# learningmatter-mit/surface-sampling

Hardware: AMD Instinct MI355X
Metric: MC energy-evaluations/sec (SrTiO3(001) ~250-atom slabs, 3-model PaiNN ensemble E+F incl. neighbor list) (higher is better)
Workload: dtype f32 via fp16x2-split MFMA (3 products), fp32 accumulate; neighbor decisions f64; 1 GPU; SrTiO3(001) PaiNN x3, 256 batched independent chains per GPU (BASELINE configs[3]), 248-272 atoms/chain; chains_per_gpu=256, atoms_per_gpu=66503, edges_per_gpu=2747786, slots_per_gpu=2836316, models=3, streams_per_gpu=2, parallelism=one GPU, no collective

## Files before the change

surface-sampling_amd/csrc/api_batch.hip:

```cpp
#include <cmath>

#include "ewald_dev.h"

namespace vssr {

static void cell_host_setup(const double *cell, const uint8_t *pbc, double cutoff, double inv[9], int nimg[3],
                            bool &ok) {
    const double *a = cell, *b = cell + 3, *c = cell + 6;
    double bc[3] = {b[1] * c[2] - b[2] * c[1], b[2] * c[0] - b[0] * c[2], b[0] * c[1] - b[1] * c[0]};
    double ca[3] = {c[1] * a[2] - c[2] * a[1], c[2] * a[0] - c[0] * a[2], c[0] * a[1] - c[1] * a[0]};
    double ab[3] = {a[1] * b[2] - a[2] * b[1], a[2] * b[0] - a[0] * b[2], a[0] * b[1] - a[1] * b[0]};
    double vol = a[0] * bc[0] + a[1] * bc[1] + a[2] * bc[2];
    ok = true;
    for (int x = 0; x < 9; ++x) inv[x] = 0.0;
    nimg[0] = nimg[1] = nimg[2] = 0;
    if (!(pbc[0] || pbc[1] || pbc[2])) return;
    if (std::fabs(vol) < 1e-12) { ok = false; return; }
    for (int x = 0; x < 3; ++x) { inv[x] = bc[x] / vol; inv[3 + x] = ca[x] / vol; inv[6 + x] = ab[x] / vol; }
    double hgt[3] = {std::fabs(vol) / std::sqrt(bc[0] * bc[0] + bc[1] * bc[1] + bc[2] * bc[2]),
                     std::fabs(vol) / std::sqrt(ca[0] * ca[0] + ca[1] * ca[1] + ca[2] * ca[2]),
                     std::fabs(vol) / std::sqrt(ab[0] * ab[0] + ab[1] * ab[1] + ab[2] * ab[2])};
    for (int k = 0; k < 3; ++k)
        if (pbc[k]) nimg[k] = (int)std::floor(cutoff / hgt[k]) + 1;
}
// ... 66 lines not shown
        }
        h->ew_stride = (int)stride;
        if (h->d_ew_S.ensure(sizeof(double) * 2 * (size_t)n_cfg * (size_t)(stride + 1)))
            return set_err(h, VSSR_E_NOMEM, "k-space structure factors: out of device memory");
    }
    if (h->d_pos.ensure(sizeof(double) * 3 * N) || h->d_Z.ensure(sizeof(int) * N) ||
        h->d_atom_cfg.ensure(sizeof(int) * N) || h->d_cfg_start.ensure(sizeof(int) * (n_cfg + 1)) ||
        h->d_cell.ensure(sizeof(double) * 9 * n_cfg) || h->d_invcell.ensure(sizeof(double) * 9 * n_cfg) ||
        h->d_nimg.ensure(sizeof(int) * 3 * n_cfg) || h->d_pbc.ensure((size_t)3 * n_cfg))
        return set_err(h, VSSR_E_NOMEM, "batch buffers: out of device memory");
    VSSR_HIP(h, hipMemcpy(h->d_pos.p, pos, sizeof(double) * 3 * N, hipMemcpyHostToDevice));
    VSSR_HIP(h, hipMemcpy(h->d_Z.p, Z, sizeof(int) * N, hipMemcpyHostToDevice));
    VSSR_HIP(h, hipMemcpy(h->d_atom_cfg.p, atom_cfg.data(), sizeof(int) * N, hipMemcpyHostToDevice));
    VSSR_HIP(h, hipMemcpy(h->d_cfg_start.p, start.data(), sizeof(int) * (n_cfg + 1), hipMemcpyHostToDevice));
    VSSR_HIP(h, hipMemcpy(h->d_cell.p, cell, sizeof(double) * 9 * n_cfg, hipMemcpyHostToDevice));
    VSSR_HIP(h, hipMemcpy(h->d_invcell.p, inv.data(), sizeof(double) * 9 * n_cfg, hipMemcpyHostToDevice));
    VSSR_HIP(h, hipMemcpy(h->d_nimg.p, nimg.data(), sizeof(int) * 3 * n_cfg, hipMemcpyHostToDevice));
    VSSR_HIP(h, hipMemcpy(h->d_pbc.p, pbc, (size_t)3 * n_cfg, hipMemcpyHostToDevice));
    h->n_cfg = n_cfg;
    h->n_atoms = N;
    if (h->kind == Kind::PAINN) {
        std::vector<int> zmap(h->n_embed, -1), zlist;
        for (int i = 0; i < N; ++i)
            if (zmap[Z[i]] < 0) { zmap[Z[i]] = 1; }
        for (int z = 0; z < h->n_embed; ++z)
            if (zmap[z] > 0) { zmap[z] = (int)zlist.size(); zlist.push_back(z); }
        h->l0_nz = (int)zlist.size() <= L0_MAX_SPECIES ? (int)zlist.size() : 0;
        if (h->d_zmap.ensure(sizeof(int) * h->n_embed) || h->d_zlist.ensure(sizeof(int) * (zlist.size() + 1)))
            return set_err(h, VSSR_E_NOMEM, "species tables");
        VSSR_HIP(h, hipMemcpy(h->d_zmap.p, zmap.data(), sizeof(int) * h->n_embed, hipMemcpyHostToDevice));
        VSSR_HIP(h, hipMemcpy(h->d_zlist.p, zlist.data(), sizeof(int) * zlist.size(), hipMemcpyHostToDevice));
    }
    h->max_cfg_atoms = 0;
    for (int b = 0; b < n_cfg; ++b) h->max_cfg_atoms = n_atoms[b] > h->max_cfg_atoms ? n_atoms[b] : h->max_cfg_atoms;
    if (h->kind == Kind::PAINN) {
        const bool bundles = (size_t)h->max_cfg_atoms * sizeof(int) <= 48 * 1024;
        std::vector<unsigned char> bcls(n_cfg);
        std::vector<int> lists[EDGE_MFMA_CLASSES], blists[EDGE_MFMA_BCLASSES];
        for (int c = 0; c < EDGE_CLASSES; ++c) { h->n_class[c] = 0; h->max_class_atoms[c] = 0; }
        for (int c = 0; c < EDGE_BCLASSES; ++c) { h->n_bclass[c] = 0; h->max_bclass_atoms[c] = 0; }
        for (int b = 0; b < n_cfg; ++b) {
            int c = (h->edge_impl && bundles) ? edge_class_of(n_atoms[b]) : EDGE_CLASS_GATHER;
            int bc = (h->edge_impl && bundles) ? edge_bclass_of(n_atoms[b]) : EDGE_BCLASS_GATHER;
            if (c <= EDGE_CLASS_FS16M && h->fs16_max_atoms >= 0 && n_atoms[b] > h->fs16_max_atoms) c = EDGE_CLASS_FS8;
            if (bc == EDGE_BCLASS_FS16 && h->fs16_max_atoms >= 0 && n_atoms[b] > h->fs16_max_atoms) bc = EDGE_BCLASS_FS8;
            if (c == EDGE_CLASS_FS8 && h->fs8_max_atoms >= 0 && n_atoms[b] > h->fs8_max_atoms) { c = EDGE_CLASS_FS4; bc = EDGE_BCLASS_FS4; }
            if (h->fwd_two_pass == 16 && c == EDGE_CLASS_FS8 && edge_class_of(n_atoms[b]) == EDGE_CLASS_FS8) c = EDGE_CLASS_FS4;
            if (bc != EDGE_BCLASS_GATHER && ((h->bwd_multi_pass == 1 && edge_bclass_of(n_atoms[b]) != EDGE_BCLASS_FS16) || h->bwd_multi_pass == 2))
                bc = EDGE_BCLASS_FS16P;
            bcls[b] = (unsigned char)bc;
            h->n_class[c] += 1;
            h->n_bclass[bc] += 1;
            if (n_atoms[b] > h->max_class_atoms[c]) h->max_class_atoms[c] = n_atoms[b];
            if (n_atoms[b] > h->max_bclass_atoms[bc]) h->max_bclass_atoms[bc] = n_atoms[b];
            if (c != EDGE_CLASS_GATHER) lists[c].push_back(b);
            if (bc != EDGE_BCLASS_GATHER) blists[bc].push_back(b);
        }
        std::vector<int> cat;
        for (int c = 0; c < EDGE_MFMA_CLASSES; ++c) cat.insert(cat.end(), lists[c].begin(), lists[c].end());
        for (int c = 0; c < EDGE_MFMA_BCLASSES; ++c) cat.insert(cat.end(), blists[c].begin(), blists[c].end());
        cat.push_back(0);
        const std::vector<unsigned char> &cls = bcls;
        if (h->d_chain_class.ensure((size_t)n_cfg) || h->d_class_list.ensure(sizeof(int) * cat.size()))
            return set_err(h, VSSR_E_NOMEM, "chain class tables");
        VSSR_HIP(h, hipMemcpy(h->d_chain_class.p, cls.data(), (size_t)n_cfg, hipMemcpyHostToDevice));
        VSSR_HIP(h, hipMemcpy(h->d_class_list.p, cat.data(), sizeof(int) * cat.size(), hipMemcpyHostToDevice));
    }
// ... 492 lines not shown
```

surface-sampling_amd/csrc/api_painn.hip:

```cpp
#include <cmath>

#include "vssr_internal.h"

namespace vssr {

static void transpose(const float *src, int rows, int cols, float *dst) {
    for (int r = 0; r < rows; ++r)
        for (int c = 0; c < cols; ++c) dst[(size_t)c * rows + r] = src[(size_t)r * cols + c];
}

static int upload_weights(vssr_handle *h, const vssr_painn_config *cfg) {
    const int M = cfg->n_models, L = cfg->num_conv, R = cfg->n_rbf, H = cfg->readout_hidden, NE = cfg->n_embed;
    const size_t per_layer = (size_t)F * F + F + (size_t)F3 * F + F3 + (size_t)F3 * R + F3 + 2 * (size_t)F * F +
                             (size_t)F * 2 * F + F + (size_t)F3 * F + F3;
    const size_t blob_len = (size_t)NE * F + L * per_layer + (size_t)H * F + H + H + 1;
    if (cfg->weights_len != blob_len)
        return set_err(h, VSSR_E_BADARG, "weights_len %llu does not match the layout (%zu floats)",
                       (unsigned long long)cfg->weights_len, blob_len);
    const size_t t_per_layer = (size_t)F * F + (size_t)F * F3 + 2 * (size_t)F * F + (size_t)2 * F * F + (size_t)F * F3;
    const size_t img_len = blob_len + L * t_per_layer + (size_t)F * H;
    std::vector<float> img(img_len * M);
    std::vector<ModelW> table(M);
    if (h->weights.ensure(img.size() * sizeof(float)))
        return set_err(h, VSSR_E_NOMEM, "weights: out of device memory");
// ... 104 lines not shown
            const float *W1 = hb + o; o += (size_t)F * F;
            const float *b1 = hb + o; o += F;
            const float *W2 = hb + o; o += (size_t)F3 * F;
            const float *b2 = hb + o; o += F3;
            const float *Wd = hb + o; o += (size_t)F3 * R;
            const float *bd = hb + o;
            l0_build_tables(hb, W1, b1, W2, b2, Wd, bd, NE, A.data() + per_model * m, At.data() + per_model * m);
        }
        const size_t pk = l0_packed_dwords(NE);
        std::vector<unsigned> A16(pk * M), At16(pk * M);
        for (int m = 0; m < M; ++m) l0_pack_tables(A.data() + per_model * m, NE, A16.data() + pk * m, At16.data() + pk * m);
        if (h->d_l0A.ensure(A16.size() * sizeof(unsigned)) || h->d_l0At.ensure(At16.size() * sizeof(unsigned)))
            return set_err(h, VSSR_E_NOMEM, "layer-0 tables");
        VSSR_HIP(h, hipMemcpy(h->d_l0A.p, A16.data(), A16.size() * sizeof(unsigned), hipMemcpyHostToDevice));
        VSSR_HIP(h, hipMemcpy(h->d_l0At.p, At16.data(), At16.size() * sizeof(unsigned), hipMemcpyHostToDevice));
    }
    if (h->model_table.ensure(sizeof(ModelW) * M)) return set_err(h, VSSR_E_NOMEM, "model table");
    VSSR_HIP(h, hipMemcpy(h->model_table.p, table.data(), sizeof(ModelW) * M, hipMemcpyHostToDevice));
    return VSSR_OK;
}

static void read_env_knobs(vssr_handle *h) {
    if (const char *e = getenv("VSSR_PAINN_PATH")) h->painn_general = h->painn_general || strcmp(e, "general") == 0;
    if (const char *e = getenv("VSSR_EDGE_IMPL")) h->edge_impl = (strcmp(e, "gather") == 0) ? 0 : 1;
    if (const char *e = getenv("VSSR_L0_FACTORISE")) h->l0_enabled = atoi(e);
    if (h->painn_general) h->l0_enabled = 0;
    if (const char *e = getenv("VSSR_UPD_SAVE")) h->upd_save = atoi(e);
    if (const char *e = getenv("VSSR_DEBUG_KEEP")) h->debug_keep = atoi(e);
    if (const char *e = getenv("VSSR_EDGE_FS16_MAX")) h->fs16_max_atoms = atoi(e);
    if (const char *e = getenv("VSSR_EDGE_FS8_MAX")) h->fs8_max_atoms = atoi(e);
    if (const char *e = getenv("VSSR_EDGE_BWD_MPASS")) h->bwd_multi_pass = atoi(e);
    if (const char *e = getenv("VSSR_EDGE_SUB_CHUNK")) { const int c = atoi(e); if (c >= 8) { h->sub_chunk_fwd = c; h->sub_chunk_bwd = c; } }
    if (const char *e = getenv("VSSR_EDGE_FWD_2PASS")) { const int w = atoi(e); h->fwd_two_pass = (w == 8 || w == 16) ? w : w ? 16 : 0; }
}

}

using namespace vssr;

extern "C" {

int vssr_create(const vssr_painn_config *cfg, vssr_handle **out) {
    if (!cfg || !out) return set_err(nullptr, VSSR_E_BADARG, "null argument");
    *out = nullptr;
    if (cfg->struct_size != sizeof(vssr_painn_config))
        return set_err(nullptr, VSSR_E_BADARG, "vssr_painn_config size mismatch (%u vs %zu)", cfg->struct_size,
                       sizeof(vssr_painn_config));
    if (cfg->feat_dim < 16 || cfg->feat_dim > 256 || cfg->feat_dim % 16 != 0 || cfg->n_rbf < 1 || cfg->n_rbf > 32)
        return set_err(nullptr, VSSR_E_BADARG,
                       "feat_dim must be a multiple of 16 in 16..256 and n_rbf in 1..32 (got %d, %d)", cfg->feat_dim, cfg->n_rbf);
    if (cfg->n_models < 1 || cfg->n_models > MAX_MODELS || cfg->num_conv < 1 || cfg->num_conv > MAX_LAYERS ||
        cfg->readout_hidden < 1 || cfg->readout_hidden > F || cfg->n_embed < 1 || !cfg->weights ||
        !(cfg->cutoff > 0) || !(cfg->model_units_per_ev > 0))
        return set_err(nullptr, VSSR_E_BADARG, "bad PaiNN configuration");
    if (cfg->excl_vol && (cfg->excl_power < 1 || cfg->excl_power > 64 || !(cfg->excl_sigma > 0)))
        return set_err(nullptr, VSSR_E_BADARG, "excluded volume: power %d (1 .. 64) / sigma %g out of range", cfg->excl_power,
                       (double)cfg->excl_sigma);
    return create_handle(Kind::PAINN, cfg->device, out, [cfg](vssr_handle *h) {
        h->n_models = cfg->n_models; h->n_rbf = cfg->n_rbf; h->num_conv = cfg->num_conv; h->n_embed = cfg->n_embed;
        h->readout_hidden = cfg->readout_hidden; h->cutoff = cfg->cutoff; h->excl_vol = cfg->excl_vol;
        h->excl_power = cfg->excl_power; h->excl_sigma = cfg->excl_sigma; h->units_per_ev = cfg->model_units_per_ev;
        h->feat_dim = cfg->feat_dim;
        h->painn_general = !(cfg->feat_dim == F && cfg->n_rbf == 20);
        read_env_knobs(h);
        int rc = VSSR_OK;
        if (h->painn_general)
// ... 21 lines not shown
```

surface-sampling_amd/csrc/nbr.hip:

```cpp
#include "nbr_dev.h"

namespace vssr {

__global__ void k_wrap(int n, const double *__restrict__ pos, const int *__restrict__ atom_cfg,
                       const double *__restrict__ cell, const double *__restrict__ invcell,
                       const uint8_t *__restrict__ pbc, double *__restrict__ wpos, int *__restrict__ wrap) {
    int i = blockIdx.x * blockDim.x + threadIdx.x;
    if (i >= n) return;
    wrap_atom(i, pos, atom_cfg, cell, invcell, pbc, wpos, wrap);
}

template <bool FILL, int LPC>
__global__ void __launch_bounds__(256)
k_nbr(int n, const double *__restrict__ wpos, const int *__restrict__ atom_cfg,
      const int *__restrict__ cfg_start, const double *__restrict__ cell, const double *__restrict__ invcell,
      const int *__restrict__ nimg, double rc2, int *__restrict__ deg, const int *__restrict__ row_start, float4 *__restrict__ edge,
      int *__restrict__ edge_S, long long slot_cap, unsigned long long *__restrict__ hits_buf, int hits_stride,
      const unsigned char *__restrict__ active) {
    const int i = blockIdx.x * (256 / LPC) + threadIdx.x / LPC;
    if (i >= n) return;
    nbr_row<FILL, LPC>(i, wpos, atom_cfg, cfg_start, cell, invcell, nimg, rc2, deg, row_start, edge, edge_S, slot_cap, hits_buf, hits_stride,
                       active);
}

struct ScanTile {
    int d[4], pd[4], p, real;
};
__device__ __forceinline__ ScanTile scan_tile_load(int n, const int *__restrict__ deg, int i0) {
    ScanTile s;
    if (i0 + 3 < n) {
        const int4 v = *reinterpret_cast<const int4 *>(deg + i0);
        s.d[0] = v.x; s.d[1] = v.y; s.d[2] = v.z; s.d[3] = v.w;
    } else {
#pragma unroll
        for (int u = 0; u < 4; ++u) s.d[u] = i0 + u < n ? deg[i0 + u] : 0;
    }
#pragma unroll
    for (int u = 0; u < 4; ++u) s.pd[u] = i0 + u < n ? max((s.d[u] + 3) & ~3, 8) : 0;
    s.p = s.pd[0] + s.pd[1] + s.pd[2] + s.pd[3];
    s.real = s.d[0] + s.d[1] + s.d[2] + s.d[3];
    return s;
}

__global__ void __launch_bounds__(1024)
k_scan_tiles(int n, const int *__restrict__ deg, int *__restrict__ tile_sums ) {
    __shared__ int wsum[16], wreal[16];
    const int t = threadIdx.x, lane = t & 63, w = t >> 6;
    const ScanTile s = scan_tile_load(n, deg, blockIdx.x * 4096 + 4 * t);
    const int x = wave_incl_scan_i32(s.p), xr = wave_incl_scan_i32(s.real);
    if (lane == 63) { wsum[w] = x; wreal[w] = xr; }
    __syncthreads();
    if (t == 0) {
        int a = 0, b = 0;
#pragma unroll
// ... 31 lines not shown
    __syncthreads();
    run = 0; run_real = 0;
    int woff = 0;
#pragma unroll
    for (int k = 0; k < 16; ++k) {
        run += wrun[k];
        run_real += wrun_real[k];
        if (k < w) woff += wsum[k];
    }
    const int i0 = tile * 4096 + 4 * t;
    int o = (int)(run + woff + x - s.p);
#pragma unroll
    for (int u = 0; u < 4; ++u) {
        if (i0 + u < n) row_start[i0 + u] = o;
        o += s.pd[u];
    }
    if (last && t == 0) {
        long long own = 0, own_real = 0;
        if (tile_sums) { own = tile_sums[2 * tile]; own_real = tile_sums[2 * tile + 1]; }
        else {
            for (int k = 0; k < 16; ++k) { own += wsum[k]; own_real += wreal[k]; }
        }
        const long long total = run + own, total_real = run_real + own_real;
        row_start[n] = (int)total;
        counters[0] = (int)total;
        counters[1] = (int)total_real;
        counters[2] = (total > slot_cap - 64 || total > 2147483000LL) ? 1 : 0;
    }
}

template <int LPC>
__global__ void __launch_bounds__(256)
k_rev(int n, const int *__restrict__ row_start, const float4 *__restrict__ edge,
      const int *__restrict__ edge_S, int *__restrict__ rev, const int *__restrict__ counters, ActiveView av) {
    const int i = blockIdx.x * (256 / LPC) + threadIdx.x / LPC;
    if (i >= n || counters[2] || !av.atom(i)) return;
    rev_row<LPC>(i, row_start, edge, edge_S, rev);
}

__device__ __forceinline__ void split2_f16(float x, unsigned &h, unsigned &l) {
    const _Float16 hh = (_Float16)x;
    const _Float16 ll = (_Float16)(x - (float)hh);
    h = __builtin_bit_cast(unsigned short, hh);
    l = __builtin_bit_cast(unsigned short, ll);
}
__device__ __forceinline__ size_t f16_unit(size_t slot, int kq, int piece) {
    return (slot >> 2) * 32 + (size_t)piece * 16 + (size_t)kq * 4 + (slot & 3);
}
__device__ __forceinline__ void write_f16_record(const float (&v)[5], float env, uint4 *__restrict__ tab, size_t slot, int kq,
                                                 float spare, unsigned jbits) {
    unsigned h[6], l[6];
#pragma unroll
    for (int k = 0; k < 5; ++k) split2_f16(v[k], h[k], l[k]);
    split2_f16(env, h[5], l[5]);
    auto pk = [](unsigned lo, unsigned hi) { return lo | (hi << 16); };
    const unsigned env_piece = kq == 0 ? l[5] : kq == 3 ? 0u : h[5];
    tab[f16_unit(slot, kq, 0)] = make_uint4(pk(l[0], l[1]), pk(l[2], l[3]), pk(l[4], env_piece), pk(h[0], h[1]));
    tab[f16_unit(slot, kq, 1)] = make_uint4(pk(h[2], h[3]), pk(h[4], h[4]), __float_as_uint(spare), jbits);
}

__device__ __forceinline__ float quarter_class_sum(float x) {
    x += __builtin_bit_cast(float, __builtin_amdgcn_update_dpp(0, __builtin_bit_cast(int, x), 0x124, 0xF, 0xF, true));
    x += __builtin_bit_cast(float, __builtin_amdgcn_update_dpp(0, __builtin_bit_cast(int, x), 0x128, 0xF, 0xF, true));
    const unsigned u = __float_as_uint(x);
    const auto r32 = __builtin_amdgcn_permlane32_swap(u, u, false, false);
    const float y = __uint_as_float(r32[0]) + __uint_as_float(r32[1]);
    const unsigned v = __float_as_uint(y);
    const auto r16 = __builtin_amdgcn_permlane16_swap(v, v, false, false);
    return __uint_as_float(r16[0]) + __uint_as_float(r16[1]);
}
// ... 193 lines not shown
                first[p * n + c] = f;
                if (any && p > 0) atomicAdd(&cnt[p], 1);
                kprev = k;
            }
        }
    }
    __syncthreads();
    if (threadIdx.x >= 1 && threadIdx.x < SUB_MAX_PASSES) n_entries[(size_t)(threadIdx.x - 1) * n_cfg + b] = cnt[threadIdx.x];
    unsigned *keys = reinterpret_cast<unsigned *>(sdeg + 2 * SUB_MAX_PASSES * n);
    for (int p = 0; p < P; ++p) {
        const int *lp = len + p * n;
        __syncthreads();
        for (int c = threadIdx.x; c < BSORT_N; c += blockDim.x) keys[c] = c < n ? ((unsigned)(4095 - min(lp[c], 4095)) << 11) | (unsigned)c : 0xFFFFFFFFu;
        __syncthreads();
        lds_bitonic_sort(keys);
        for (int r = threadIdx.x; r < n; r += blockDim.x) {
            const int c = (int)(keys[r] & 2047u);
            bundle_sub[(size_t)p * N + a0 + r] = make_int4(c, row_start[a0 + c] + first[p * n + c], lp[c], 0);
        }
    }
}

int build_neighbors(vssr_handle *h, double cutoff) {
    const int n = h->n_atoms;
    hipStream_t st = h->stream;
    if (h->d_wpos.ensure(sizeof(double) * 3 * n) || h->d_wrap.ensure(sizeof(int) * 3 * n) ||
        h->d_deg.ensure(sizeof(int) * n) || h->d_row_start.ensure(sizeof(int) * (n + 1)) ||
        h->d_counters.ensure(sizeof(int) * 4) || h->d_tile_sums.ensure(sizeof(int) * 2 * ((size_t)n / 4096 + 1)))
        return set_err(h, VSSR_E_NOMEM, "neighbor buffers: out of device memory");
    if (h->slot_cap < (int64_t)n * h->cap_per_atom + 64) h->slot_cap = (int64_t)n * h->cap_per_atom + 64;
    if (h->d_edge.ensure(sizeof(float4) * h->slot_cap) || h->d_edge_S.ensure(sizeof(int) * h->slot_cap) ||
        h->d_rev.ensure(sizeof(int) * h->slot_cap))
        return set_err(h, VSSR_E_NOMEM, "edge buffers: out of device memory");
    unsigned long long *hits_buf = nullptr;
    const int hits_stride = (h->max_cfg_atoms + 63) & ~63;
    if (h->max_images <= 64 && (size_t)n * hits_stride * 8 <= ((size_t)1 << 30) &&
        !h->d_hits.ensure((size_t)n * hits_stride * 8))
        hits_buf = h->d_hits.as<unsigned long long>();
    h->prof.begin(KC_NBR, st);
    dim3 blk(128), grd((n + 127) / 128);
    const int lpc_rev = h->kind != Kind::PAINN ? 16 : 32;
    dim3 wblk(256);
    auto grid_for = [&](int lpc) { return dim3((n + 256 / lpc - 1) / (256 / lpc)); };
#define NBR_ARGS(FILLING) n, h->d_wpos.as<double>(), h->d_atom_cfg.as<int>(), h->d_cfg_start.as<int>(), h->d_cell.as<double>(),          \
        h->d_invcell.as<double>(), h->d_nimg.as<int>(), cutoff * cutoff, h->d_deg.as<int>(),                                            \
        (FILLING) ? h->d_row_start.as<int>() : (const int *)nullptr, (FILLING) ? h->d_edge.as<float4>() : (float4 *)nullptr,            \
        (FILLING) ? h->d_edge_S.as<int>() : (int *)nullptr, (FILLING) ? (long long)h->slot_cap : (long long)0, hits_buf, hits_stride,   \
        h->active_mask
    hipLaunchKernelGGL(k_wrap, grd, blk, 0, st, n, h->d_pos.as<double>(), h->d_atom_cfg.as<int>(),
                       h->d_cell.as<double>(), h->d_invcell.as<double>(), h->d_pbc.as<uint8_t>(),
                       h->d_wpos.as<double>(), h->d_wrap.as<int>());
    hipLaunchKernelGGL((k_nbr<false, 16>), grid_for(16), wblk, 0, st, NBR_ARGS(false));
    const int n_tiles = n > 0 ? (n + 4095) / 4096 : 1;
    if (n_tiles > 1)
        hipLaunchKernelGGL(k_scan_tiles, dim3(n_tiles), dim3(1024), 0, st, n, h->d_deg.as<int>(), h->d_tile_sums.as<int>());
    hipLaunchKernelGGL(k_scan_rows, dim3(n_tiles), dim3(1024), 0, st, n, h->d_deg.as<int>(),
                       h->d_row_start.as<int>(), h->d_counters.as<int>(), (long long)h->slot_cap,
                       n_tiles > 1 ? h->d_tile_sums.as<int>() : (const int *)nullptr);
    hipLaunchKernelGGL((k_nbr<true, 16>), grid_for(16), wblk, 0, st, NBR_ARGS(true));
#undef NBR_ARGS
    const ActiveView rev_av{h->active_mask, h->d_atom_cfg.as<int>()};
#define REV_ARGS n, h->d_row_start.as<int>(), h->d_edge.as<float4>(), h->d_edge_S.as<int>(), h->d_rev.as<int>(), h->d_counters.as<int>(), rev_av
    if (lpc_rev == 16) hipLaunchKernelGGL(k_rev<16>, grid_for(16), wblk, 0, st, REV_ARGS);
    else hipLaunchKernelGGL(k_rev<32>, grid_for(32), wblk, 0, st, REV_ARGS);
#undef REV_ARGS
    if (h->kind == Kind::PAINN && !h->painn_general) {
        const int nzf = (h->l0_enabled && h->l0_nz >= 1 && h->l0_nz <= 4) ? h->l0_nz : 0;
        const bool want_f32 = h->l0_enabled && nzf == 0;
        if ((want_f32 && (h->d_erec.ensure(sizeof(float4) * h->slot_cap) || h->d_rho.ensure(sizeof(float) * 24 * h->slot_cap))) ||
            h->d_dist.ensure(sizeof(float2) * h->slot_cap) ||
            h->d_rho16.ensure(sizeof(uint4) * 8 * h->slot_cap) || h->d_drho16.ensure(sizeof(uint4) * 8 * h->slot_cap) ||
            h->d_zslot.ensure((size_t)h->slot_cap) || h->d_bundle.ensure(sizeof(int4) * (size_t)n) ||
            h->d_excl.ensure(sizeof(float) * (size_t)n))
            return set_err(h, VSSR_E_NOMEM, "edge geometry tables: out of device memory");
        const void *tabs[2] = {h->d_rho16.as<uint4>(), h->d_drho16.as<uint4>()};
        bool cleared = h->zero_entry_cap == h->slot_cap;
        for (int k = 0; k < 2; ++k) cleared = cleared && h->zero_entry_tab[k] == tabs[k];
        if (!cleared) {
            VSSR_HIP(h, hipMemsetAsync(h->d_rho16.as<uint4>() + 32 * (size_t)((h->slot_cap >> 2) - 1), 0, 32 * sizeof(uint4), st));
            VSSR_HIP(h, hipMemsetAsync(h->d_drho16.as<uint4>() + 32 * (size_t)((h->slot_cap >> 2) - 1), 0, 32 * sizeof(uint4), st));
            h->zero_entry_cap = h->slot_cap;
            for (int k = 0; k < 2; ++k) h->zero_entry_tab[k] = tabs[k];
        }
        if (nzf && h->d_l0T.ensure(sizeof(float) * (size_t)n * nzf * 96))
            return set_err(h, VSSR_E_NOMEM, "layer-0 factorisation buffers: out of device memory");
        h->l0T_by_geom = nzf > 0;
#define LAUNCH_GEOM(NZ)                                                                                                          \
        hipLaunchKernelGGL(k_edge_geom<NZ>, dim3(n), dim3(64), 0, st, n, h->d_row_start.as<int>(), h->d_atom_cfg.as<int>(),      \
                           h->d_cfg_start.as<int>(), h->d_edge.as<float4>(), h->d_counters.as<int>(), h->cutoff,               \
                           h->excl_sigma, h->excl_power, want_f32 ? h->d_erec.as<float4>() : (float4 *)nullptr,                \
                           want_f32 ? h->d_rho.as<float>() : (float *)nullptr, h->d_dist.as<float2>(), h->d_rho16.as<uint4>(), \
                           h->d_drho16.as<uint4>(), h->d_Z.as<int>(), h->d_zmap.as<int>(), h->d_zslot.as<unsigned char>(),     \
                           h->d_excl.as<float>(), h->active_mask, nzf ? h->d_l0T.as<float>() : (float *)nullptr)
        switch (nzf) {
            case 1: LAUNCH_GEOM(1); break;
// ... 47 lines not shown
```

surface-sampling_amd/csrc/nbr_dev.h:

```cpp
#ifndef VSSR_NBR_DEV_H
#define VSSR_NBR_DEV_H
#include "vssr_internal.h"

namespace vssr {

__device__ inline int pack_shift(int s0, int s1, int s2) {
    return ((s0 + 128) & 255) | (((s1 + 128) & 255) << 8) | (((s2 + 128) & 255) << 16);
}
__device__ inline void unpack_shift(int p, int &s0, int &s1, int &s2) {
    s0 = (p & 255) - 128;
    s1 = ((p >> 8) & 255) - 128;
    s2 = ((p >> 16) & 255) - 128;
}

__device__ __forceinline__ void wrap_atom(int i, const double *__restrict__ pos, const int *__restrict__ atom_cfg,
                                          const double *__restrict__ cell, const double *__restrict__ invcell,
                                          const uint8_t *__restrict__ pbc, double *__restrict__ wpos, int *__restrict__ wrap) {
    int c = atom_cfg[i];
    const double *C = cell + 9 * c, *I = invcell + 9 * c;
    double p[3] = {pos[3 * i], pos[3 * i + 1], pos[3 * i + 2]};
    double q[3] = {p[0], p[1], p[2]};
    for (int a = 0; a < 3; ++a) {
        int w = 0;
        if (pbc[3 * c + a]) {
            double f = I[3 * a] * p[0] + I[3 * a + 1] * p[1] + I[3 * a + 2] * p[2];
            w = (int)floor(f);
            q[0] -= w * C[3 * a];
            q[1] -= w * C[3 * a + 1];
            q[2] -= w * C[3 * a + 2];
        }
        wrap[3 * i + a] = w;
    }
    wpos[3 * i] = q[0];
    wpos[3 * i + 1] = q[1];
    wpos[3 * i + 2] = q[2];
}

template <int LPC>
__device__ __forceinline__ int group_excl_scan(int v, int &total) {
    if constexpr (LPC == 64) {
        const int x = wave_incl_scan_i32(v);
        total = __builtin_amdgcn_readlane(x, 63);
        return x - v;
    } else {
        static_assert(LPC == 16 || LPC == 32, "a wave, half a wave or one 16-lane row per centre");
        int x = v;
        x += __builtin_amdgcn_update_dpp(0, x, 0x111, 0xF, 0xF, true);
        x += __builtin_amdgcn_update_dpp(0, x, 0x112, 0xF, 0xF, true);
        x += __builtin_amdgcn_update_dpp(0, x, 0x114, 0xF, 0xF, true);
        x += __builtin_amdgcn_update_dpp(0, x, 0x118, 0xF, 0xF, true);
        if constexpr (LPC == 32) x += __builtin_amdgcn_update_dpp(0, x, 0x142, 0xA, 0xF, false);
        total = __shfl(x, (threadIdx.x & 63) | (LPC - 1));
        return x - v;
    }
}

template <bool FILL, int LPC>
__device__ __forceinline__ void nbr_row(int i, const double *__restrict__ wpos, const int *__restrict__ atom_cfg,
      const int *__restrict__ cfg_start, const double *__restrict__ cell, const double *__restrict__ invcell,
      const int *__restrict__ nimg, double rc2, int *__restrict__ deg, const int *__restrict__ row_start, float4 *__restrict__ edge,
      int *__restrict__ edge_S, long long slot_cap, unsigned long long *__restrict__ hits_buf, int hits_stride,
      const unsigned char *__restrict__ active) {
    const int lane = threadIdx.x & (LPC - 1);
    const int c = atom_cfg[i];
    if (active && !active[c]) {
        if (!FILL && lane == 0) deg[i] = 0;
        return;
    }
    const int a0 = cfg_start[c], a1 = cfg_start[c + 1];
    const double *C = cell + 9 * c;
    const int n0 = nimg[3 * c], n1 = nimg[3 * c + 1], n2 = nimg[3 * c + 2];
    const double C0 = C[0], C1 = C[1], C2 = C[2], C3 = C[3], C4 = C[4], C5 = C[5], C6 = C[6], C7 = C[7], C8 = C[8];
    const double px = wpos[3 * i], py = wpos[3 * i + 1], pz = wpos[3 * i + 2];
    const double *I = invcell + 9 * c;
    const double I0 = I[0], I1 = I[1], I2 = I[2], I3 = I[3], I4 = I[4], I5 = I[5], I6 = I[6], I7 = I[7], I8 = I[8];
    const double rcut = sqrt(rc2);
    const double wd0 = rcut * sqrt(I0 * I0 + I1 * I1 + I2 * I2) * (1.0 + 1e-9) + 1e-9;
    const double wd1 = rcut * sqrt(I3 * I3 + I4 * I4 + I5 * I5) * (1.0 + 1e-9) + 1e-9;
    const double wd2 = rcut * sqrt(I6 * I6 + I7 * I7 + I8 * I8) * (1.0 + 1e-9) + 1e-9;
    long long base = FILL ? (long long)row_start[i] : 0;
    int run = 0;
    for (int j0 = a0; j0 < a1; j0 += LPC) {
        const int j = j0 + lane;
        const bool have = j < a1;
        double bx = 0, by = 0, bz = 0;
        if (have) { bx = wpos[3 * j] - px; by = wpos[3 * j + 1] - py; bz = wpos[3 * j + 2] - pz; }
        int cnt = 0;
        unsigned long long hits = 0ull;
        unsigned long long *hslot = hits_buf ? hits_buf + (size_t)i * hits_stride + (j - a0) : nullptr;
        if (FILL && hslot) {
            if (have) {
                hits = *hslot;
                cnt = __builtin_popcountll(hits);
            }
        } else if (have) {
            const double f0 = I0 * bx + I1 * by + I2 * bz, f1 = I3 * bx + I4 * by + I5 * bz, f2 = I6 * bx + I7 * by + I8 * bz;
            const int lo0 = n0 ? max(-n0, (int)ceil(-wd0 - f0)) : 0, hi0 = n0 ? min(n0, (int)floor(wd0 - f0)) : 0;
            const int lo1 = n1 ? max(-n1, (int)ceil(-wd1 - f1)) : 0, hi1 = n1 ? min(n1, (int)floor(wd1 - f1)) : 0;
            const int lo2 = n2 ? max(-n2, (int)ceil(-wd2 - f2)) : 0, hi2 = n2 ? min(n2, (int)floor(wd2 - f2)) : 0;
            const int iw1 = 2 * n1 + 1, iw2 = 2 * n2 + 1;
            for (int s0 = lo0; s0 <= hi0; ++s0)
                for (int s1 = lo1; s1 <= hi1; ++s1)
                    for (int s2 = lo2; s2 <= hi2; ++s2) {
                        const int img = ((s0 + n0) * iw1 + (s1 + n1)) * iw2 + (s2 + n2);
                        if (i == j && s0 == 0 && s1 == 0 && s2 == 0) continue;
                        double rx = bx + s0 * C0 + s1 * C3 + s2 * C6;
                        double ry = by + s0 * C1 + s1 * C4 + s2 * C7;
                        double rz = bz + s0 * C2 + s1 * C5 + s2 * C8;
                        double d2 = rx * rx + ry * ry + rz * rz;
                        if (d2 <= rc2 && d2 > 0.0) {
                            ++cnt;
                            if (img < 64) hits |= 1ull << img;
                        }
                    }
            if (!FILL && hslot) *hslot = hits;
        }
        int total;
        const int off = group_excl_scan<LPC>(cnt, total);
        if (FILL && cnt > 0) {
            long long slot = base + run + off;
            const int w1 = 2 * n1 + 1, w2 = 2 * n2 + 1;
            if ((2 * n0 + 1) * w1 * w2 <= 64) {
                while (hits) {
                    const int img = __builtin_ctzll(hits);
                    hits &= hits - 1;
                    const int s0 = img / (w1 * w2) - n0, s1 = (img / w2) % w1 - n1, s2 = img % w2 - n2;
                    const double rx = bx + s0 * C0 + s1 * C3 + s2 * C6;
                    const double ry = by + s0 * C1 + s1 * C4 + s2 * C7;
                    const double rz = bz + s0 * C2 + s1 * C5 + s2 * C8;
                    if (slot < slot_cap) {
                        edge[slot] = make_float4((float)rx, (float)ry, (float)rz, __int_as_float(j));
                        edge_S[slot] = pack_shift(s0, s1, s2);
                    }
                    ++slot;
                }
            } else {
                for (int s0 = -n0; s0 <= n0; ++s0)
                    for (int s1 = -n1; s1 <= n1; ++s1)
                        for (int s2 = -n2; s2 <= n2; ++s2) {
                            if (i == j && s0 == 0 && s1 == 0 && s2 == 0) continue;
                            double rx = bx + s0 * C0 + s1 * C3 + s2 * C6;
                            double ry = by + s0 * C1 + s1 * C4 + s2 * C7;
                            double rz = bz + s0 * C2 + s1 * C5 + s2 * C8;
                            double d2 = rx * rx + ry * ry + rz * rz;
                            if (d2 > rc2 || d2 <= 0.0) continue;
                            if (slot < slot_cap) {
                                edge[slot] = make_float4((float)rx, (float)ry, (float)rz, __int_as_float(j));
                                edge_S[slot] = pack_shift(s0, s1, s2);
// ... 14 lines not shown
    } else if (lane == 0) {
        deg[i] = run;
    }
}

template <int LPC>
__device__ __forceinline__ void rev_row(int i, const int *__restrict__ row_start, const float4 *__restrict__ edge,
                                        const int *__restrict__ edge_S, int *__restrict__ rev) {
    const int lane = threadIdx.x & (LPC - 1);
    for (int e = row_start[i] + lane; e < row_start[i + 1]; e += LPC) {
        int j = __float_as_int(edge[e].w);
        int found = -1;
        if (j >= 0) {
            int s0, s1, s2;
            unpack_shift(edge_S[e], s0, s1, s2);
            const int want = pack_shift(-s0, -s1, -s2);
            int lo = row_start[j], hi = row_start[j + 1];
            const int row_end = hi;
            while (lo < hi) {
                const int mid = (lo + hi) >> 1;
                const int jm = __float_as_int(edge[mid].w);
                if (jm >= 0 && jm < i) lo = mid + 1; else hi = mid;
            }
            for (int e2 = lo; e2 < row_end && __float_as_int(edge[e2].w) == i; ++e2)
                if (edge_S[e2] == want) {
                    found = e2;
                    break;
                }
        }
        rev[e] = found;
    }
}

}
#endif
```

surface-sampling_amd/csrc/vssr_internal.h:

```cpp
#pragma once

#include <hip/hip_runtime.h>

#include <cstdint>
#include <cstdio>
#include <cstdlib>
#include <cstring>
#include <memory>
#include <string>
#include <utility>
#include <vector>

#include "../../include/vssr_eval.h"

namespace vssr {

constexpr int F = 128;
constexpr int F3 = 3 * F;
constexpr int MAX_LAYERS = 4;
constexpr int MAX_MODELS = 8;
constexpr int RB_MAX = 24;
constexpr int NODE_TILE = 8;
constexpr int L0_MAX_SPECIES = 8;

// ... 234 lines not shown
    DevBuf pts;
    DevBuf cen[2], siz[2], cid[2];
    DevBuf nn, flag, blk, rec, counters;
};

enum class Kind : int {
    NONE = 0,
    PAINN = 1,
    TERSOFF = 2,
    EAM = 3,
    SW = 4,
    GMM = 5,
    GMM_FIT = 6,
    CLUSTER = 7,
    PAIR = 8,
    COUNT
};
constexpr unsigned kind_bit(Kind k) { return 1u << (int)k; }
constexpr unsigned KINDS_EVAL = kind_bit(Kind::PAINN) | kind_bit(Kind::TERSOFF) | kind_bit(Kind::EAM) | kind_bit(Kind::SW) |
                                kind_bit(Kind::PAIR);

}

struct vssr_handle {
    vssr::Kind kind = vssr::Kind::NONE;
    vssr_eam_grid eam_grid = {0, 0, 0.0, 0.0, 0.0};
    int eam_nel = 0, eam_fs = 0;
    int device = 0;
    vssr::OwnedStream stream;
    std::string err;
    vssr::Profiler prof;

    int edge_impl = 1;
    int max_cfg_atoms = 0;
    vssr::DevBuf d_chain_class, d_class_list;
    int n_class[5] = {0, 0, 0, 0, 0}, max_class_atoms[5] = {0, 0, 0, 0, 0};
    int n_bclass[5] = {0, 0, 0, 0, 0}, max_bclass_atoms[5] = {0, 0, 0, 0, 0};
    int fs16_max_atoms = -1, fs8_max_atoms = -1;
    int max_images = 0;

    int n_models = 0, n_rbf = 20, num_conv = 3, n_embed = 100, readout_hidden = 64;
    int feat_dim = vssr::F;
    bool painn_general = false;
    float cutoff = 5.f;
    int excl_vol = 1, excl_power = 12;
    float excl_sigma = 1.5f;
    double units_per_ev = 1.0;
    bool has_offset = false;
    double offset_const = 0.0;

    vssr::DevBuf weights;
    vssr::DevBuf wd16;
    vssr::DevBuf node16;
    vssr::DevBuf model_table;
    vssr::DevBuf offset_per_z;

    int n_types = 0;
    double pot_cutoff = 0;
    bool ew_on = false;
    double ew_g = 0, ew_kcut = 0, ew_q[8] = {0, 0, 0, 0, 0, 0, 0, 0};
    int ew_stride = 0;
    vssr::DevBuf d_ew_S;
    vssr::DevBuf pot_params;

    bool batch_valid = false, ran = false;
    int n_cfg = 0, n_atoms = 0;
    std::vector<int> h_n_atoms, h_cfg_start;
// ... 205 lines not shown
```

Baseline: 24580 evaluations/s.

## Stage per-chain reverse-edge search in LDS and narrow neighbor hit-mask words

Adds a per-chain reverse-edge kernel that runs one 1024-thread block per chain. It loads that chain's edge keys and row offsets into up to 128 KiB of dynamic LDS, then does the binary search for each reverse edge there instead of in global memory. The per-row kernel skips chains that fit in LDS. Separately, the neighbor-list image-hit bitmask buffer now uses 16-bit or 32-bit words when the image count allows, which cuts write and read traffic between the count and fill passes. The LDS path only turns on above an atom-count threshold and can lower occupancy because of its large shared-memory footprint.

```diff
diff --git a/surface-sampling_amd/csrc/api_batch.hip b/surface-sampling_amd/csrc/api_batch.hip
--- a/surface-sampling_amd/csrc/api_batch.hip
+++ b/surface-sampling_amd/csrc/api_batch.hip
@@ -122,7 +122,11 @@
         VSSR_HIP(h, hipMemcpy(h->d_zlist.p, zlist.data(), sizeof(int) * zlist.size(), hipMemcpyHostToDevice));
     }
     h->max_cfg_atoms = 0;
-    for (int b = 0; b < n_cfg; ++b) h->max_cfg_atoms = n_atoms[b] > h->max_cfg_atoms ? n_atoms[b] : h->max_cfg_atoms;
+    h->min_cfg_atoms = n_cfg > 0 ? n_atoms[0] : 0;
+    for (int b = 0; b < n_cfg; ++b) {
+        h->max_cfg_atoms = n_atoms[b] > h->max_cfg_atoms ? n_atoms[b] : h->max_cfg_atoms;
+        h->min_cfg_atoms = n_atoms[b] < h->min_cfg_atoms ? n_atoms[b] : h->min_cfg_atoms;
+    }
     if (h->kind == Kind::PAINN) {
         const bool bundles = (size_t)h->max_cfg_atoms * sizeof(int) <= 48 * 1024;
         std::vector<unsigned char> bcls(n_cfg);
diff --git a/surface-sampling_amd/csrc/api_painn.hip b/surface-sampling_amd/csrc/api_painn.hip
--- a/surface-sampling_amd/csrc/api_painn.hip
+++ b/surface-sampling_amd/csrc/api_painn.hip
@@ -160,6 +160,7 @@
     if (const char *e = getenv("VSSR_EDGE_BWD_MPASS")) h->bwd_multi_pass = atoi(e);
     if (const char *e = getenv("VSSR_EDGE_SUB_CHUNK")) { const int c = atoi(e); if (c >= 8) { h->sub_chunk_fwd = c; h->sub_chunk_bwd = c; } }
     if (const char *e = getenv("VSSR_EDGE_FWD_2PASS")) { const int w = atoi(e); h->fwd_two_pass = (w == 8 || w == 16) ? w : w ? 16 : 0; }
+    if (const char *e = getenv("VSSR_REV_LDS_BYTES")) { const int b = atoi(e); h->rev_lds_budget = b < 0 ? 0 : b > 160 * 1024 ? 160 * 1024 : b; h->rev_lds_forced = true; }
 }
 
 }
diff --git a/surface-sampling_amd/csrc/nbr.hip b/surface-sampling_amd/csrc/nbr.hip
--- a/surface-sampling_amd/csrc/nbr.hip
+++ b/surface-sampling_amd/csrc/nbr.hip
@@ -10,16 +10,16 @@
     wrap_atom(i, pos, atom_cfg, cell, invcell, pbc, wpos, wrap);
 }
 
-template <bool FILL, int LPC>
+template <bool FILL, int LPC, class HW>
 __global__ void __launch_bounds__(256)
 k_nbr(int n, const double *__restrict__ wpos, const int *__restrict__ atom_cfg,
       const int *__restrict__ cfg_start, const double *__restrict__ cell, const double *__restrict__ invcell,
       const int *__restrict__ nimg, double rc2, int *__restrict__ deg, const int *__restrict__ row_start, float4 *__restrict__ edge,
-      int *__restrict__ edge_S, long long slot_cap, unsigned long long *__restrict__ hits_buf, int hits_stride,
+      int *__restrict__ edge_S, long long slot_cap, HW *__restrict__ hits_buf, int hits_stride,
       const unsigned char *__restrict__ active) {
     const int i = blockIdx.x * (256 / LPC) + threadIdx.x / LPC;
     if (i >= n) return;
-    nbr_row<FILL, LPC>(i, wpos, atom_cfg, cfg_start, cell, invcell, nimg, rc2, deg, row_start, edge, edge_S, slot_cap, hits_buf, hits_stride,
+    nbr_row<FILL, LPC, HW>(i, wpos, atom_cfg, cfg_start, cell, invcell, nimg, rc2, deg, row_start, edge, edge_S, slot_cap, hits_buf, hits_stride,
                        active);
 }
 
@@ -117,10 +117,27 @@
 template <int LPC>
 __global__ void __launch_bounds__(256)
 k_rev(int n, const int *__restrict__ row_start, const float4 *__restrict__ edge,
-      const int *__restrict__ edge_S, int *__restrict__ rev, const int *__restrict__ counters, ActiveView av) {
+      const int *__restrict__ edge_S, int *__restrict__ rev, const int *__restrict__ counters, ActiveView av,
+      const int *__restrict__ cfg_start, int lds_budget) {
     const int i = blockIdx.x * (256 / LPC) + threadIdx.x / LPC;
     if (i >= n || counters[2] || !av.atom(i)) return;
+    if (lds_budget > 0) {
+        const int c = av.atom_cfg[i], a0 = cfg_start[c], a1 = cfg_start[c + 1];
+        if (rev_chain_fits(row_start[a1] - row_start[a0], a1 - a0, lds_budget)) return;
+    }
     rev_row<LPC>(i, row_start, edge, edge_S, rev);
+}
+
+constexpr int REV_CHAIN_THREADS = 1024;
+__global__ void __launch_bounds__(REV_CHAIN_THREADS)
+k_rev_chain(const int *__restrict__ cfg_start, const int *__restrict__ row_start, const float4 *__restrict__ edge,
+            const int *__restrict__ edge_S, int *__restrict__ rev, const int *__restrict__ counters, ActiveView av, int lds_budget) {
+    extern __shared__ int rev_lds[];
+    const int c = blockIdx.x;
+    if (counters[2] || !av.chain(c)) return;
+    const int a0 = cfg_start[c], a1 = cfg_start[c + 1], s0 = row_start[a0], s1 = row_start[a1];
+    if (!rev_chain_fits(s1 - s0, a1 - a0, lds_budget)) return;
+    rev_chain(a0, a1, s0, s1, row_start, edge, edge_S, rev, rev_lds);
 }
 
 __device__ __forceinline__ void split2_f16(float x, unsigned &h, unsigned &l) {
@@ -380,11 +397,14 @@
     if (h->d_edge.ensure(sizeof(float4) * h->slot_cap) || h->d_edge_S.ensure(sizeof(int) * h->slot_cap) ||
         h->d_rev.ensure(sizeof(int) * h->slot_cap))
         return set_err(h, VSSR_E_NOMEM, "edge buffers: out of device memory");
-    unsigned long long *hits_buf = nullptr;
+    void *hits_buf = nullptr;
     const int hits_stride = (h->max_cfg_atoms + 63) & ~63;
-    if (h->max_images <= 64 && (size_t)n * hits_stride * 8 <= ((size_t)1 << 30) &&
-        !h->d_hits.ensure((size_t)n * hits_stride * 8))
-        hits_buf = h->d_hits.as<unsigned long long>();
+    size_t hits_word = h->max_images <= 16 ? 2 : h->max_images <= 32 ? 4 : 8;
+    if (h->max_images <= 64 && (size_t)n * hits_stride * hits_word <= ((size_t)1 << 30) &&
+        !h->d_hits.ensure((size_t)n * hits_stride * hits_word))
+        hits_buf = h->d_hits.p;
+    else
+        hits_word = 8;
     h->prof.begin(KC_NBR, st);
     dim3 blk(128), grd((n + 127) / 128);
     const int lpc_rev = h->kind != Kind::PAINN ? 16 : 32;
@@ -393,22 +413,43 @@
 #define NBR_ARGS(FILLING) n, h->d_wpos.as<double>(), h->d_atom_cfg.as<int>(), h->d_cfg_start.as<int>(), h->d_cell.as<double>(),          \
         h->d_invcell.as<double>(), h->d_nimg.as<int>(), cutoff * cutoff, h->d_deg.as<int>(),                                            \
         (FILLING) ? h->d_row_start.as<int>() : (const int *)nullptr, (FILLING) ? h->d_edge.as<float4>() : (float4 *)nullptr,            \
-        (FILLING) ? h->d_edge_S.as<int>() : (int *)nullptr, (FILLING) ? (long long)h->slot_cap : (long long)0, hits_buf, hits_stride,   \
+        (FILLING) ? h->d_edge_S.as<int>() : (int *)nullptr, (FILLING) ? (long long)h->slot_cap : (long long)0, (HW *)hits_buf, hits_stride,   \
         h->active_mask
     hipLaunchKernelGGL(k_wrap, grd, blk, 0, st, n, h->d_pos.as<double>(), h->d_atom_cfg.as<int>(),
                        h->d_cell.as<double>(), h->d_invcell.as<double>(), h->d_pbc.as<uint8_t>(),
                        h->d_wpos.as<double>(), h->d_wrap.as<int>());
-    hipLaunchKernelGGL((k_nbr<false, 16>), grid_for(16), wblk, 0, st, NBR_ARGS(false));
+#define LAUNCH_NBR(FILLING)                                                                                                             \
+    do {                                                                                                                                \
+        if (hits_word == 2) { using HW = uint16_t; hipLaunchKernelGGL((k_nbr<FILLING, 16, HW>), grid_for(16), wblk, 0, st, NBR_ARGS(FILLING)); }      \
+        else if (hits_word == 4) { using HW = uint32_t; hipLaunchKernelGGL((k_nbr<FILLING, 16, HW>), grid_for(16), wblk, 0, st, NBR_ARGS(FILLING)); } \
+        else { using HW = unsigned long long; hipLaunchKernelGGL((k_nbr<FILLING, 16, HW>), grid_for(16), wblk, 0, st, NBR_ARGS(FILLING)); }           \
+    } while (0)
+    LAUNCH_NBR(false);
     const int n_tiles = n > 0 ? (n + 4095) / 4096 : 1;
     if (n_tiles > 1)
         hipLaunchKernelGGL(k_scan_tiles, dim3(n_tiles), dim3(1024), 0, st, n, h->d_deg.as<int>(), h->d_tile_sums.as<int>());
     hipLaunchKernelGGL(k_scan_rows, dim3(n_tiles), dim3(1024), 0, st, n, h->d_deg.as<int>(),
                        h->d_row_start.as<int>(), h->d_counters.as<int>(), (long long)h->slot_cap,
                        n_tiles > 1 ? h->d_tile_sums.as<int>() : (const int *)nullptr);
-    hipLaunchKernelGGL((k_nbr<true, 16>), grid_for(16), wblk, 0, st, NBR_ARGS(true));
+    LAUNCH_NBR(true);
+#undef LAUNCH_NBR
 #undef NBR_ARGS
     const ActiveView rev_av{h->active_mask, h->d_atom_cfg.as<int>()};
-#define REV_ARGS n, h->d_row_start.as<int>(), h->d_edge.as<float4>(), h->d_edge_S.as<int>(), h->d_rev.as<int>(), h->d_counters.as<int>(), rev_av
+    constexpr int REV_CHAIN_MIN_ATOMS = 24576;
+    const bool rev_chain_on = h->kind == Kind::PAINN && (long long)h->min_cfg_atoms * 68 + 4 <= (long long)h->rev_lds_budget &&
+                              (h->rev_lds_forced || n >= REV_CHAIN_MIN_ATOMS);
+    const int rev_budget = rev_chain_on ? h->rev_lds_budget : 0;
+    if (rev_budget > 0) {
+        if (!h->rev_lds_attr) {
+            VSSR_HIP(h, hipFuncSetAttribute((const void *)k_rev_chain, hipFuncAttributeMaxDynamicSharedMemorySize, 160 * 1024));
+            h->rev_lds_attr = true;
+        }
+        hipLaunchKernelGGL(k_rev_chain, dim3(h->n_cfg), dim3(REV_CHAIN_THREADS), (size_t)rev_budget, st, h->d_cfg_start.as<int>(),
+                           h->d_row_start.as<int>(), h->d_edge.as<float4>(), h->d_edge_S.as<int>(), h->d_rev.as<int>(), h->d_counters.as<int>(),
+                           rev_av, rev_budget);
+    }
+#define REV_ARGS n, h->d_row_start.as<int>(), h->d_edge.as<float4>(), h->d_edge_S.as<int>(), h->d_rev.as<int>(), h->d_counters.as<int>(), rev_av, \
+        h->d_cfg_start.as<int>(), rev_budget
     if (lpc_rev == 16) hipLaunchKernelGGL(k_rev<16>, grid_for(16), wblk, 0, st, REV_ARGS);
     else hipLaunchKernelGGL(k_rev<32>, grid_for(32), wblk, 0, st, REV_ARGS);
 #undef REV_ARGS
diff --git a/surface-sampling_amd/csrc/nbr_dev.h b/surface-sampling_amd/csrc/nbr_dev.h
--- a/surface-sampling_amd/csrc/nbr_dev.h
+++ b/surface-sampling_amd/csrc/nbr_dev.h
@@ -55,11 +55,11 @@
     }
 }
 
-template <bool FILL, int LPC>
+template <bool FILL, int LPC, class HW = unsigned long long>
 __device__ __forceinline__ void nbr_row(int i, const double *__restrict__ wpos, const int *__restrict__ atom_cfg,
       const int *__restrict__ cfg_start, const double *__restrict__ cell, const double *__restrict__ invcell,
       const int *__restrict__ nimg, double rc2, int *__restrict__ deg, const int *__restrict__ row_start, float4 *__restrict__ edge,
-      int *__restrict__ edge_S, long long slot_cap, unsigned long long *__restrict__ hits_buf, int hits_stride,
+      int *__restrict__ edge_S, long long slot_cap, HW *__restrict__ hits_buf, int hits_stride,
       const unsigned char *__restrict__ active) {
     const int lane = threadIdx.x & (LPC - 1);
     const int c = atom_cfg[i];
@@ -87,7 +87,7 @@
         if (have) { bx = wpos[3 * j] - px; by = wpos[3 * j + 1] - py; bz = wpos[3 * j + 2] - pz; }
         int cnt = 0;
         unsigned long long hits = 0ull;
-        unsigned long long *hslot = hits_buf ? hits_buf + (size_t)i * hits_stride + (j - a0) : nullptr;
+        HW *hslot = hits_buf ? hits_buf + (size_t)i * hits_stride + (j - a0) : nullptr;
         if (FILL && hslot) {
             if (have) {
                 hits = *hslot;
@@ -113,7 +113,7 @@
                             if (img < 64) hits |= 1ull << img;
                         }
                     }
-            if (!FILL && hslot) *hslot = hits;
+            if (!FILL && hslot) *hslot = (HW)hits;
         }
         int total;
         const int off = group_excl_scan<LPC>(cnt, total);
@@ -194,5 +194,50 @@
     }
 }
 
+__device__ __forceinline__ bool rev_chain_fits(int n_slots, int n_atoms, int budget) {
+    return budget > 0 && (long long)n_slots * 8 + (long long)(n_atoms + 1) * 4 <= (long long)budget;
+}
+
+__device__ __forceinline__ void rev_chain(int a0, int a1, int s0, int s1, const int *__restrict__ row_start,
+                                          const float4 *__restrict__ edge, const int *__restrict__ edge_S, int *__restrict__ rev,
+                                          int *__restrict__ lds) {
+    const int ns = s1 - s0, na = a1 - a0;
+    int2 *keys = reinterpret_cast<int2 *>(lds);
+    int *rows = lds + 2 * ns;
+    for (int e = threadIdx.x; e < ns; e += blockDim.x) keys[e] = make_int2(__float_as_int(edge[s0 + e].w), edge_S[s0 + e]);
+    for (int k = threadIdx.x; k <= na; k += blockDim.x) rows[k] = row_start[a0 + k] - s0;
+    __syncthreads();
+    const int lane = threadIdx.x & 15;
+    for (int il = threadIdx.x >> 4; il < na; il += blockDim.x >> 4) {
+        const int i = a0 + il;
+        for (int e = rows[il] + lane; e < rows[il + 1]; e += 16) {
+            const int2 key = keys[e];
+            const int j = key.x;
+            int found = -1;
+            if (j >= 0) {
+                int t0, t1, t2;
+                unpack_shift(key.y, t0, t1, t2);
+                const int want = pack_shift(-t0, -t1, -t2);
+                int lo = rows[j - a0], hi = rows[j - a0 + 1];
+                const int row_end = hi;
+                while (lo < hi) {
+                    const int mid = (lo + hi) >> 1;
+                    const int jm = keys[mid].x;
+                    if (jm >= 0 && jm < i) lo = mid + 1; else hi = mid;
+                }
+                for (int e2 = lo; e2 < row_end; ++e2) {
+                    const int2 k2 = keys[e2];
+                    if (k2.x != i) break;
+                    if (k2.y == want) {
+                        found = s0 + e2;
+                        break;
+                    }
+                }
+            }
+            rev[s0 + e] = found;
+        }
+    }
+}
+
 }
 #endif
diff --git a/surface-sampling_amd/csrc/vssr_internal.h b/surface-sampling_amd/csrc/vssr_internal.h
--- a/surface-sampling_amd/csrc/vssr_internal.h
+++ b/surface-sampling_amd/csrc/vssr_internal.h
@@ -290,7 +290,10 @@
     vssr::Profiler prof;
 
     int edge_impl = 1;
-    int max_cfg_atoms = 0;
+    int max_cfg_atoms = 0, min_cfg_atoms = 0;
+    int rev_lds_budget = 128 * 1024;
+    bool rev_lds_forced = false;
+    bool rev_lds_attr = false;
     vssr::DevBuf d_chain_class, d_class_list;
     int n_class[5] = {0, 0, 0, 0, 0}, max_class_atoms[5] = {0, 0, 0, 0, 0};
     int n_bclass[5] = {0, 0, 0, 0, 0}, max_bclass_atoms[5] = {0, 0, 0, 0, 0};
```

After: 24680 evaluations/s, median of 6. No clear change (+0.4%).
